# hydradarpa/kalman-hydra

Measured on AMD Instinct MI355X. Metric: frames/sec (Brox flow + EKF update) at 1024^2, higher is better.
Workload: dtype f32 (flow, renders) / f64 (EKF sums and state)

## Files before the change

include/hydra_mi.h:

```cpp
#ifndef HYDRA_MI_H
#define HYDRA_MI_H

#include <stdint.h>

#ifdef __cplusplus
extern "C" {
#endif

#define HM_OK 0
#define HM_ERR_ARG (-1)
#define HM_ERR_HIP (-2)
#define HM_ERR_STATE (-3)
#define HM_ERR_NUMERIC (-4)

const char *hm_last_error(void);
const char *hm_version(void);
int hm_device_count(void);

int hm_dev_alloc(int device, uint64_t bytes, void **out);
int hm_dev_free(int device, void *ptr);
int hm_dev_upload(int device, void *dst, const void *src, uint64_t bytes);
int hm_dev_download(int device, void *dst, const void *src, uint64_t bytes);
int hm_copy_stream_create(int device, void **stream_out);
int hm_copy_stream_destroy(int device, void *stream);
// ... 50 lines not shown
int hm_ctx_destroy(hm_ctx_t h);
int hm_set_texture(hm_ctx_t h, const uint8_t *tex);
int hm_set_observation(hm_ctx_t h, const uint8_t *y_im, const float *y_fx,
                       const float *y_fy, const uint8_t *y_m);
int hm_set_observation_dev(hm_ctx_t h, const uint8_t *d_y_im, const float *d_y_fx,
                           const float *d_y_fy, const uint8_t *d_y_m);

int hm_render(hm_ctx_t h, const double *X, uint8_t *im, float *fx, float *fy, uint8_t *m);


int hm_initjacobian(hm_ctx_t h, const double *X, int masked);
int hm_jz(hm_ctx_t h, const double *Xp, int masked, double *jz, double jzc[4]);
int hm_j(hm_ctx_t h, const double *X, double deltaX, int i, int j, double *out);
int hm_jz_multi(hm_ctx_t h, const double *Xp, int masked, const int32_t *labels, int n_labels,
                double *hz, double *hzc);
int hm_j_multi(hm_ctx_t h, const double *X, double deltaX, int n_pairs, const int32_t *ee,
               const int32_t *labels, int n_labels, double *hsum, double *nz, double *hcomp);
int hm_project_mask(hm_ctx_t h, const uint8_t *y_m, double *X, int *moved);
int hm_prune_mask(hm_ctx_t h, const uint8_t *y_m, uint8_t *out);
int hm_error(hm_ctx_t h, const double *X, int masked, double err[4], float *fx, float *fy);

int hm_measure(hm_ctx_t h, const double *X, double deltaX, int masked,
               double *Hz, double *Hzc, double *HTH);
int hm_update_begin(hm_ctx_t h, const double *W_prior, const double *X0);
int hm_update_prefactor(hm_ctx_t h);
int hm_update_step(hm_ctx_t h, const double *X, double deltaX, int masked, double *step, double *Hzc,
                   double err[4]);
int hm_update_cov(hm_ctx_t h, int which, double *W_out);
int hm_update_run(hm_ctx_t h, const double *W_prior, double *X, double deltaX, int masked, int max_iter,
                  double reltol, int info[4], double *errs, double *Hzc, double *gains, double *W_out);
int hm_cov_fetch(hm_ctx_t h, double *W_out);
int hm_ms_newton(int n_vertices, int n_bars, const int32_t *bars, const double *l0, double kappa, double M,
                 double dt, int maxiter, double tol, double *X, int *newton_iterations);
int hm_ms_worker_create(void **worker);
int hm_ms_worker_destroy(void *worker);
int hm_ms_newton_start(void *worker, int n_vertices, int n_bars, const int32_t *bars, const double *l0, double kappa,
                       double M, double dt, int maxiter, double tol, const double *X);
int hm_ms_newton_finish(void *worker, double *X, int *newton_iterations);
int hm_ms_worker_attach(void *worker, hm_ctx_t ctx);
int hm_newton_dev_start(hm_ctx_t h, int N, int n_bars, const int32_t *bars, const double *l0, double kappa, double M,
                        double dt, int maxiter, double tol, const double *X);
int hm_newton_dev_finish(hm_ctx_t h, double *X, int *newton_iterations);
int hm_update_arm_newton(hm_ctx_t h, void *worker, int n_bars, const int32_t *bars, const double *l0, double kappa,
                         double M, double dt, int maxiter, double tol);
int hm_update_arm_cov(hm_ctx_t h, double eps_F);
int hm_predict_take(hm_ctx_t h, const double *X, int n_bars, const int32_t *bars, const double *l0, double kappa,
// ... 69 lines not shown
```

kalman-hydra_amd/_lib.py:

```python
import ctypes
import os

import numpy as np

_HERE = os.path.dirname(os.path.abspath(__file__))
SO_PATH = os.environ.get("HYDRA_MI_SO") or os.path.join(_HERE, "libhydra_mi.so")

c_f32p = ctypes.POINTER(ctypes.c_float)
c_f64p = ctypes.POINTER(ctypes.c_double)
c_u8p = ctypes.POINTER(ctypes.c_uint8)
c_i32p = ctypes.POINTER(ctypes.c_int32)
c_vp = ctypes.c_void_p

SIGNATURES = {
    "hm_last_error": (ctypes.c_char_p, []),
    "hm_version": (ctypes.c_char_p, []),
    "hm_device_count": (ctypes.c_int, []),
    "hm_dev_alloc": (ctypes.c_int, [ctypes.c_int, ctypes.c_uint64, ctypes.POINTER(c_vp)]),
    "hm_dev_free": (ctypes.c_int, [ctypes.c_int, c_vp]),
    "hm_dev_upload": (ctypes.c_int, [ctypes.c_int, c_vp, c_vp, ctypes.c_uint64]),
    "hm_dev_download": (ctypes.c_int, [ctypes.c_int, c_vp, c_vp, ctypes.c_uint64]),
    "hm_copy_stream_create": (ctypes.c_int, [ctypes.c_int, ctypes.POINTER(c_vp)]),
    "hm_copy_stream_destroy": (ctypes.c_int, [ctypes.c_int, c_vp]),
    "hm_copy_stream_sync": (ctypes.c_int, [ctypes.c_int, c_vp]),
# ... 23 lines not shown
    "hm_op_pyr_down": (ctypes.c_int, [c_vp, ctypes.c_int, ctypes.c_int, ctypes.c_float, c_vp, ctypes.c_int, ctypes.c_int]),
    "hm_op_deriv_all": (ctypes.c_int, [c_vp, c_vp, ctypes.c_int, ctypes.c_int, ctypes.POINTER(c_vp)]),
    "hm_op_add_prolong": (ctypes.c_int, [c_vp, c_vp, c_vp, c_vp, ctypes.c_int, ctypes.c_int, c_vp, c_vp, ctypes.c_int,
                                         ctypes.c_int]),
    "hm_op_warp": (ctypes.c_int, [ctypes.POINTER(c_vp), ctypes.c_int, ctypes.c_int, ctypes.POINTER(c_vp), ctypes.c_int]),
    "hm_op_prepare": (ctypes.c_int, [ctypes.POINTER(c_vp), ctypes.c_int, ctypes.c_int, ctypes.c_float,
                                     ctypes.c_float, ctypes.POINTER(c_vp)]),
    "hm_op_sor": (ctypes.c_int, [c_vp, c_vp, ctypes.POINTER(c_vp), ctypes.c_int, ctypes.c_int, ctypes.c_int,
                                 ctypes.c_int, ctypes.c_float]),
    "hm_ctx_create": (ctypes.c_int, [ctypes.c_int, ctypes.c_int, ctypes.c_int, ctypes.c_int, ctypes.c_int, c_vp,
                                     c_vp, ctypes.c_double, ctypes.c_double, ctypes.c_double, ctypes.POINTER(c_vp)]),
    "hm_ctx_destroy": (ctypes.c_int, [c_vp]),
    "hm_set_texture": (ctypes.c_int, [c_vp, c_vp]),
    "hm_set_observation": (ctypes.c_int, [c_vp, c_vp, c_vp, c_vp, c_vp]),
    "hm_set_observation_dev": (ctypes.c_int, [c_vp, c_vp, c_vp, c_vp, c_vp]),
    "hm_render": (ctypes.c_int, [c_vp, c_vp, c_vp, c_vp, c_vp, c_vp]),
    "hm_initjacobian": (ctypes.c_int, [c_vp, c_vp, ctypes.c_int]),
    "hm_jz": (ctypes.c_int, [c_vp, c_vp, ctypes.c_int, c_f64p, c_f64p]),
    "hm_j": (ctypes.c_int, [c_vp, c_vp, ctypes.c_double, ctypes.c_int, ctypes.c_int, c_f64p]),
    "hm_jz_multi": (ctypes.c_int, [c_vp, c_vp, ctypes.c_int, c_vp, ctypes.c_int, c_vp, c_vp]),
    "hm_j_multi": (ctypes.c_int, [c_vp, c_vp, ctypes.c_double, ctypes.c_int, c_vp, c_vp, ctypes.c_int, c_vp, c_vp, c_vp]),
    "hm_error": (ctypes.c_int, [c_vp, c_vp, ctypes.c_int, c_f64p, c_vp, c_vp]),
    "hm_measure": (ctypes.c_int, [c_vp, c_vp, ctypes.c_double, ctypes.c_int, c_vp, c_vp, c_vp]),
    "hm_update_begin": (ctypes.c_int, [c_vp, c_vp, c_vp]),
    "hm_update_step": (ctypes.c_int, [c_vp, c_vp, ctypes.c_double, ctypes.c_int, c_vp, c_vp, c_f64p]),
    "hm_update_cov": (ctypes.c_int, [c_vp, ctypes.c_int, c_vp]),
    "hm_update_prefactor": (ctypes.c_int, [c_vp]),
    "hm_update_run": (ctypes.c_int, [c_vp, c_vp, c_vp, ctypes.c_double, ctypes.c_int, ctypes.c_int, ctypes.c_double,
                                     ctypes.POINTER(ctypes.c_int), c_vp, c_vp, c_vp, c_vp]),
    "hm_update_last_error": (ctypes.c_int, [c_vp, c_vp, c_f64p]),
    "hm_cov_fetch": (ctypes.c_int, [c_vp, c_vp]),
    "hm_project_mask": (ctypes.c_int, [c_vp, c_vp, c_vp, c_vp]),
    "hm_cov_predict": (ctypes.c_int, [c_vp, c_vp, ctypes.c_int, c_vp, c_vp, ctypes.c_double, ctypes.c_double,
                                      ctypes.c_double, c_vp]),
    "hm_ms_newton": (ctypes.c_int, [ctypes.c_int, ctypes.c_int, c_vp, c_vp, ctypes.c_double, ctypes.c_double,
                                    ctypes.c_double, ctypes.c_int, ctypes.c_double, c_vp, ctypes.POINTER(ctypes.c_int)]),
    "hm_ms_worker_create": (ctypes.c_int, [ctypes.POINTER(c_vp)]),
    "hm_ms_worker_destroy": (ctypes.c_int, [c_vp]),
    "hm_ms_newton_start": (ctypes.c_int, [c_vp, ctypes.c_int, ctypes.c_int, c_vp, c_vp, ctypes.c_double, ctypes.c_double,
                                          ctypes.c_double, ctypes.c_int, ctypes.c_double, c_vp]),
    "hm_ms_newton_finish": (ctypes.c_int, [c_vp, c_vp, ctypes.POINTER(ctypes.c_int)]),
    "hm_ms_worker_attach": (ctypes.c_int, [c_vp, c_vp]),
    "hm_newton_dev_start": (ctypes.c_int, [c_vp, ctypes.c_int, ctypes.c_int, c_vp, c_vp, ctypes.c_double, ctypes.c_double,
                                           ctypes.c_double, ctypes.c_int, ctypes.c_double, c_vp]),
    "hm_newton_dev_finish": (ctypes.c_int, [c_vp, c_vp, ctypes.POINTER(ctypes.c_int)]),
    "hm_prune_mask": (ctypes.c_int, [c_vp, c_vp, c_vp]),
# ... 154 lines not shown
```

kalman-hydra_amd/csrc/ekf.hip:

```cpp
#include "hm_common.h"
#include "ekf_kernels.h"
#include "dense_kernels.h"
#include "chol_flow_kernels.h"
#include "project_kernels.h"
#include "predict_kernels.h"
#include "view_kernels.h"
#include "body_kernels.h"
#include "roi_kernels.h"
#include "smooth_kernels.h"
#include <algorithm>
#include <atomic>
#include <chrono>
#include <cmath>
#include <condition_variable>
#include <cstring>
#include <functional>
#include <mutex>
#include <set>
#include <thread>
#include <utility>
#include <vector>

struct Helper {
    std::thread th;
// ... 50 lines not shown

struct hm_ctx {
    int device, W, H, N, T, E, njobs;
    HmOwner own{1};
    Helper helper;
    bool helper_used = false;
    int tail_async = 1;
    double eps_Z, eps_J, eps_M;
    hipStream_t stream;
    int *d_tri, *d_star_off, *d_star_tri, *d_edges;
    int *d_nb_off = nullptr, *d_nb_u = nullptr, *d_nb_e = nullptr;
    float *d_uv;
    uint8_t *d_tex;
    std::vector<int> edges;
    uint8_t *d_yim, *d_ym;
    float *d_yfx, *d_yfy, *d_yfxm, *d_yfym;
    bool obs_owned = true;
    const uint8_t *o_yim, *o_ym;
    const float *o_yfx, *o_yfy;
    bool have_tex, have_obs, have_ref;
    Targets ref, P, Q;
    TriSetup *d_setup, *d_cfgs;
    int4 *d_ubox;
    int *d_tlist = nullptr, *d_tcount = nullptr;
    unsigned *d_tmask = nullptr;
    double *d_X, *d_out, *d_partial;
    uint8_t *d_im8, *d_m8;
    std::vector<double> X0;
    double *d_HTH;
    double *d_H, *d_Hz, *d_Hzc, *d_invW0, *d_Af[2], *d_T[2], *d_step, *d_Wtmp, *d_X0, *d_Xn, *d_Wprior, *d_gain, *d_Awork, *d_Lt[2];
    std::vector<double> upd_X0;
    int upd_last = -1, upd_prev = -1;
    double *d_Wres;
    double *pin;
    size_t pin_n;
    int *pin_scratch;
    std::vector<double> resv, tailv;
    int result_delay = 0;
    bool tail_pending = false;
    bool tail_valid = false;
    long long tail_ticket = 0;
    hipStream_t tail_stream = nullptr;
    const uint8_t *armed_mask = nullptr;
    std::vector<int> sp_h_off, sp_h_bar, sp_h_other;
    std::vector<double> sp_h_blk;
    std::vector<int32_t> sp_bars_cached;
// ... 326 lines not shown
                hm_set_error("hm_ctx_create: vertex %d has %d neighbours, limit %d", v, (int)nb[v].size(), PREP_MAX_ENTRIES / 4 - 1);
                rc = HM_ERR_ARG;
            }
        }
        step(upload(h->own, &h->d_nb_off, noff.data(), noff.size()));
        step(upload(h->own, &h->d_nb_u, nu.data(), nu.size()));
        step(upload(h->own, &h->d_nb_e, ne.data(), ne.size()));
    }
    hipError_t e = hipSuccess;
    auto dev = [&](auto **p, size_t bytes) { if (e == hipSuccess) e = h->own.alloc(p, bytes); };
    if (rc == HM_OK) {
        const char *pe = getenv("HYDRA_MI_EKF_PRIORITY");
        e = h->own.stream(&h->stream, !(pe && atoi(pe) == 0));
        dev(&h->d_tex, n);
        dev(&h->d_yim, n);
        dev(&h->d_ym, n);
        dev(&h->d_yfx, n * sizeof(float));
        dev(&h->d_yfy, n * sizeof(float));
        dev(&h->d_yfxm, n * sizeof(float));
        dev(&h->d_yfym, n * sizeof(float));
        dev(&h->d_setup, (size_t)T * sizeof(TriSetup));
        dev(&h->d_cfgs, (size_t)N * MEAS_NCFG * (EKF_MAX_STAR + 1) * sizeof(TriSetup));
        dev(&h->d_ubox, (size_t)N * UBOX_STRIDE * sizeof(int4));
        dev(&h->d_tmask, (size_t)N * TMASK_STRIDE * sizeof(unsigned));
        dev(&h->d_tlist, (size_t)N * TMASK_STRIDE * sizeof(int));
        dev(&h->d_tcount, (size_t)N * sizeof(int));
        dev(&h->d_X, (size_t)4 * N * sizeof(double));
        dev(&h->d_out, (size_t)h->njobs * MEAS_VSPLIT_MAX * MEAS_OUT * sizeof(double));
        dev(&h->d_partial, (size_t)h->red_blocks * 4 * sizeof(double));
        h->ntiles = hm_cdiv(W, RI_W) * hm_cdiv(H, 8);
        dev(&h->d_tpart, (size_t)h->ntiles * RI_NV * sizeof(double));
        dev(&h->d_im8, n);
        dev(&h->d_m8, n);
        const size_t n4 = (size_t)4 * N, nn = n4 * n4 * sizeof(double);
        dev(&h->d_H, nn);
        dev(&h->d_HTH, nn);
        if (e == hipSuccess) e = hipMemsetAsync(h->d_HTH, 0, nn, h->stream);
        dev(&h->d_invW0, nn);
        const size_t nn_aug = (size_t)(hm_cdiv((int)n4, DNB) * DNB + DNB) * n4 * sizeof(double);
        dev(&h->d_Af[0], nn_aug);
        dev(&h->d_Af[1], nn_aug);
        dev(&h->d_Awork, nn_aug);
        const size_t ld_bytes = (size_t)hm_cdiv((int)n4, DNB) * DNB * DNB * sizeof(double);
        dev(&h->d_T[0], nn);
        dev(&h->d_T[1], nn);
        dev(&h->d_step, n4 * sizeof(double));
// ... 62 lines not shown
        HM_ARG(value >= 2 && value <= 2048, "hm_ctx_tune: chol_flow_wgs must be in 2..2048 (the chain workgroup and at least one task workgroup)");
        h->flow_wgs = value;
    } else if (!strcmp(key, "render_rows")) {
        HM_ARG(value == 8 || value == 16, "hm_ctx_tune: render_rows must be 8 or 16");
        h->render_rows = value;
    } else if (!strcmp(key, "chol_flow_stall")) {
        HM_ARG(value >= 0 && value <= 100000, "hm_ctx_tune: chol_flow_stall must be in 0..100000");
        h->flow_stall = value;
    } else if (!strcmp(key, "result_delay")) {
        HM_ARG(value >= 0 && value <= 5000, "hm_ctx_tune: result_delay must be in 0..5000 (microseconds)");
        h->result_delay = value;
    } else if (!strcmp(key, "tail_async")) {
        HM_ARG(value == 0 || value == 1, "hm_ctx_tune: tail_async must be 0 or 1");
        h->tail_async = value;
    } else if (!strcmp(key, "tail_split")) {
        HM_ARG(value == 0 || value == 1, "hm_ctx_tune: tail_split must be 0 or 1");
        h->tail_split = value;
    } else if (!strcmp(key, "newton_fail")) {
        HM_ARG(value == 0 || value == 1, "hm_ctx_tune: newton_fail must be 0 or 1");
        h->newton_fail = value;
    } else if (!strcmp(key, "speculate")) {
        HM_ARG(value == 0 || value == 1, "hm_ctx_tune: speculate must be 0 or 1");
        h->speculate = value;
    } else if (!strcmp(key, "edge_split")) {
        HM_ARG(value >= 1 && value <= MEAS_VSPLIT_MAX, "hm_ctx_tune: edge_split must be in 1..%d", MEAS_VSPLIT_MAX);
        h->esplit = value;
    } else if (!strcmp(key, "body_stats_cap")) {
        HM_ARG(value >= 1 && value <= BODY_STATS_CAP, "hm_ctx_tune: body_stats_cap must be in 1..%d", BODY_STATS_CAP);
        h->stats_cap = value;
    } else if (!strcmp(key, "body_rec_chunk")) {
        HM_ARG(value >= 0, "hm_ctx_tune: body_rec_chunk must be >= 0 (0: the default size)");
        h->rec_chunk = value;
    } else {
        hm_set_error("hm_ctx_tune: unknown key '%s'", key);
        return HM_ERR_ARG;
    }
    return HM_OK;
}
extern "C" void *hm_ctx_stream(hm_ctx_t h)
{
    (void)ctx_join(h);
    return h ? (void *)h->stream : nullptr;
}
extern "C" int hm_ctx_sync(hm_ctx_t h)
{
    HM_ARG(h != nullptr, "hm_ctx_sync: NULL handle");
// ... 405 lines not shown
    const int n = h->W * h->H;
    if (fx) HM_HIP(hipMemcpyAsync(fx, h->P.fx, (size_t)n * sizeof(float), hipMemcpyDeviceToHost, h->stream));
    if (fy) HM_HIP(hipMemcpyAsync(fy, h->P.fy, (size_t)n * sizeof(float), hipMemcpyDeviceToHost, h->stream));
    HM_HIP(hipMemcpyAsync(h->h_tpart.data(), h->d_tpart, (size_t)render_strips(h) * RI_NV * sizeof(double), hipMemcpyDeviceToHost, h->stream));
    HM_HIP(stream_wait(h->stream));
    double s6[RI_NV];
    hm_tile_partial_sums(h->h_tpart.data(), render_strips(h), s6);
    for (int k = 0; k < 4; k++) err[k] = s6[k];
    return HM_OK;
}

static int measure_dev(hm_ctx *h, const double *dX, bool ref_ready, double deltaX, int masked, bool regions_ready = false,
                       bool scatter = true)
{
    if (!ref_ready) {
        int rc = render_iter(h, dX, h->ref, false, masked, !regions_ready, deltaX);
        if (rc) return rc;
        regions_ready = true;
    }
    MeasureArgs a;
    measure_args(h, dX, deltaX, masked, a);
    if (!regions_ready) hipLaunchKernelGGL(k_star_regions, dim3(h->N), dim3(REGION_NT), 0, h->stream, a, h->d_area);
    hipLaunchKernelGGL(k_measure_vertex, dim3(h->N, h->vsplit), dim3(MEAS_NT), 0, h->stream, a,
                       (const TriSetup *)h->d_cfgs, (const int4 *)h->d_ubox, (const unsigned *)h->d_tmask);
    if (h->E > 0) hipLaunchKernelGGL(k_measure_edge, dim3(h->E, h->esplit), dim3(MEAS_NT), 0, h->stream, a);
    if (scatter) {
        ScatterArgs s = {h->d_out, h->d_edges, h->N, h->E, h->vsplit, h->esplit, h->eps_Z, h->eps_J, h->eps_M, deltaX, h->d_HTH, h->d_Hz, h->d_Hzc};
        hipLaunchKernelGGL(k_hth_scatter, dim3(hm_cdiv(h->njobs, 4)), dim3(256), 0, h->stream, s);
    }
    HM_HIP(hipGetLastError());
    return HM_OK;
}

static void measure_args(hm_ctx *h, const double *dX, double deltaX, int masked, MeasureArgs &a)
{
    a.m = Mesh{h->W, h->H, h->N, h->T, h->d_tri, h->d_uv, h->d_tex};
    a.topo = StarTopo{h->d_star_off, h->d_star_tri, h->d_edges, h->E};
    a.ref = h->ref;
    a.obs = obs_of(h, masked);
    a.X = dX;
    a.delta = deltaX;
    a.out = h->d_out;
    a.pool = h->pool;
    a.vsplit = h->vsplit;
    a.esplit = h->esplit;
    a.iZ = 1.0 / h->eps_Z; a.iJ = 1.0 / h->eps_J; a.iM = 1.0 / h->eps_M;
    a.cfgs = h->d_cfgs;
    a.ubox = h->d_ubox;
    a.tmask = h->d_tmask;
    a.tlist = h->d_tlist;
    a.tcount = h->d_tcount;
    a.tmask_stride = TMASK_STRIDE;
}

static int measure_on_device(hm_ctx *h, const double *X, double deltaX, int masked, bool scatter = true)
{
    HM_HIP(hipMemcpyAsync(h->d_X, X, (size_t)4 * h->N * sizeof(double), hipMemcpyHostToDevice, h->stream));
    h->X0.assign(X, X + 4 * h->N);
    h->have_ref = true;
    return measure_dev(h, h->d_X, false, deltaX, masked, false, scatter);
}

extern "C" int hm_measure(hm_ctx_t h, const double *X, double deltaX, int masked, double *Hz, double *Hzc, double *HTH)
{
    HM_ARG(h && X && Hz && HTH, "hm_measure: NULL argument");
    HM_JOIN(h);
    HM_ARG(deltaX > 0, "hm_measure: deltaX must be positive");
    NEED_TEX(h, "hm_measure");
    NEED_OBS(h, "hm_measure");
    HM_HIP(hipSetDevice(h->device));
    const size_t n4 = (size_t)4 * h->N;
    int *ovf = h->pin_scratch;
    for (int attempt = 0;; attempt++) {
        int rc = measure_on_device(h, X, deltaX, masked);
        if (rc) return rc;
        *ovf = 0;
        HM_HIP(hipMemcpyAsync(ovf, h->pool.overflow, sizeof(int), hipMemcpyDeviceToHost, h->stream));
        HM_HIP(hipStreamSynchronize(h->stream));
        if (!*ovf) break;
        if (attempt) { hm_set_error("hm_measure: the star regions do not fit the difference-image pool"); return HM_ERR_STATE; }
        rc = pool_grow(h, "hm_measure");
        if (rc) return rc;
    }
    HM_HIP(hipMemcpyAsync(Hz, h->d_Hz, n4 * sizeof(double), hipMemcpyDeviceToHost, h->stream));
    if (Hzc) HM_HIP(hipMemcpyAsync(Hzc, h->d_Hzc, n4 * 4 * sizeof(double), hipMemcpyDeviceToHost, h->stream));
    HM_HIP(hipMemcpyAsync(HTH, h->d_HTH, n4 * n4 * sizeof(double), hipMemcpyDeviceToHost, h->stream));
    HM_HIP(hipStreamSynchronize(h->stream));
    return HM_OK;
}

static int aug_rows(int n) { return hm_cdiv(n, DNB) * DNB + DNB; }

static void chol_factor(hm_ctx *h, double *A, double *L, double *Lt, double *T, double *M, int n, bool with_rhs,
                        bool first_done = false, hipStream_t st = nullptr)
{
    if (!st) st = h->stream;
    const int nb = hm_cdiv(n, DNB);
    const int nrows = with_rhs ? aug_rows(n) : n;
    const int nbr = hm_cdiv(nrows, DNB);
    if (h->chol_flow) {
        FlowArgs a = {A, L, Lt, T, h->d_flowP, n, nrows, nb, nbr, h->d_flowctl, h->flow_stall};
        if (!first_done) hipLaunchKernelGGL(k_flow_fill, dim3(nrows + FLOW_FILL_WGS), dim3(256), 0, st, a);
        hipLaunchKernelGGL(k_chol_flow, dim3(h->flow_wgs), dim3(FLOW_NT), 0, st, a);
        return;
    }
    if (!first_done) hipLaunchKernelGGL(k_chol_first, dim3(1), dim3(64), 0, st, A, Lt, n);
    for (int k = 0; k < nb; k++) {
        const int mr = nbr - k - 1, mc = std::max(nb - k - 1, 1);
        hipLaunchKernelGGL(k_chol_step, dim3((mc + k + 1) * (mr + 1)), dim3(256), 0, st, A, L, Lt, T, M, n, nrows, nb, k, mc, mc + k + 1, mr + 1);
    }
// ... 2077 lines not shown
```

kalman-hydra_amd/csrc/ekf_kernels.h:

```cpp
#pragma once
#include <hip/hip_runtime.h>
#include <stdint.h>

#define EKF_SUB 256
#define EKF_MAX_STAR 24
#define EKF_TILE 16
#define EKF_MAX_TRI 4096

struct TriSetup {
    double ea[3], eb[3], ec[3];
    double ecb[3];
    int cmin, cmax, rmin, rmax;
    int tl[3];
    float inv;
    int i0, i1, i2;
    float ux[3], uy[3], ax[3], ay[3];
};

__device__ __forceinline__ void d_tri_attr(TriSetup &s, const float *__restrict__ uv, const double *__restrict__ X, int N)
{
    const int id[3] = {s.i0, s.i1, s.i2};
    for (int k = 0; k < 3; k++) {
        s.ux[k] = uv[2 * id[k]];
        s.uy[k] = uv[2 * id[k] + 1];
// ... 468 lines not shown
{
    P.xi[pp] = make_short2(POOL_EMPTY, 0); P.yi[pp] = make_short2(0, 0);
    P.xfx[pp] = 0.0f; P.xfy[pp] = 0.0f; P.yfx[pp] = 0.0f; P.yfy[pp] = 0.0f;
    P.vxfx[pp] = 0.0f; P.vyfy[pp] = 0.0f;
}

struct MeasureArgs {
    Mesh m;
    StarTopo topo;
    Targets ref;
    Obs obs;
    const double *X;
    double delta;
    double *out;
    DPool pool;
    int vsplit;
    int esplit;
    double iZ, iJ, iM;
    TriSetup *cfgs;
    int4 *ubox;
    unsigned *tmask;
    int *tlist, *tcount;
    int tmask_stride;
};

#define MEAS_NT 256
#define MEAS_OUT 40
#define MEAS_VSPLIT_MAX 16
enum {
    A_X = 0, A_Y = 4, A_VX = 8, A_VY = 9,
    A_XX = 10, A_XY = 11, A_YY = 12,
    A_XVX = 13, A_YVX = 14,
    A_XVY = 15, A_YVY = 16,
    A_VXVX = 17, A_VYVY = 18,
    A_NV = 19
};
enum {
    B_XX = 0, B_XY = 1, B_YX = 2, B_YY = 3,
    B_XVX = 4, B_YVX = 5, B_VXX = 6, B_VXY = 7, B_VXVX = 8,
    B_XVY = 9, B_YVY = 10, B_VYX = 11, B_VYY = 12, B_VYVY = 13,
    B_NV = 14
};

#define MEAS_NCFG 5
#define UBOX_STRIDE (EKF_MAX_STAR + 4)
#define TMASK_STRIDE 1024

__device__ inline void d_vertex_cfgs(TriSetup (*cfg)[EKF_MAX_STAR + 1], int nsv, const int *trv, const Mesh &m,
                                     const double *X, int v, double d, int nthreads)
{
    const int wv = threadIdx.x >> 6, lane = threadIdx.x & 63, nw = nthreads >> 6;
    const double dxs[MEAS_NCFG] = {0, d, -d, 0, 0}, dys[MEAS_NCFG] = {0, 0, 0, d, -d};
    for (int c = wv; c < MEAS_NCFG; c += nw) d_star_setups(cfg[c], nsv, trv, m, X, v, dxs[c], dys[c], lane, 64);
}

#define REGION_NT (64 * MEAS_NCFG)
struct RegionShared {
    int4 tbox[MEAS_NCFG][EKF_MAX_STAR + 1];
    double ea[MEAS_NCFG][EKF_MAX_STAR + 1][3], eb[MEAS_NCFG][EKF_MAX_STAR + 1][3], ecb[MEAS_NCFG][EKF_MAX_STAR + 1][3];
    int box[MEAS_NCFG][4];
    int reg[4];
    int wsum[8];
};
template <int NT>
__device__ inline void d_star_regions(const MeasureArgs &a, int *__restrict__ area, int v, RegionShared &sh)
{
    const Mesh &m = a.m;
    const int nsv = a.topo.star_off[v + 1] - a.topo.star_off[v];
    const int *trv = a.topo.star_tri + a.topo.star_off[v];
    const int wv = threadIdx.x >> 6, lane = threadIdx.x & 63;
    constexpr int NW = NT / 64;
    const double d = a.delta;
    const double dxs[MEAS_NCFG] = {0, d, -d, 0, 0}, dys[MEAS_NCFG] = {0, 0, 0, d, -d};
    for (int cf = wv; cf < MEAS_NCFG; cf += NW) {
        TriSetup *dst = a.cfgs + ((size_t)v * MEAS_NCFG + cf) * (EKF_MAX_STAR + 1);
        if (lane < nsv) {
            TriSetup su;
            d_star_setup_one(su, trv[lane], m, a.X, v, dxs[cf], dys[cf]);
            dst[lane] = su;
            sh.tbox[cf][lane] = make_int4(su.cmin, su.cmax, su.rmin, su.rmax);
            for (int k = 0; k < 3; k++) { sh.ea[cf][lane][k] = su.ea[k]; sh.eb[cf][lane][k] = su.eb[k]; sh.ecb[cf][lane][k] = su.ecb[k]; }
        }
        if ((nsv & 1) && lane == 0) {
            TriSetup pad;
            d_star_setup_pad(pad);
            pad.inv = 0.0f; pad.i0 = pad.i1 = pad.i2 = 0;
            for (int k = 0; k < 3; k++) { pad.ux[k] = pad.uy[k] = pad.ax[k] = pad.ay[k] = 0.0f; }
            dst[nsv] = pad;
        }
    }
    __syncthreads();
    if (wv == 0 && lane < UBOX_STRIDE) {
        int4 u = make_int4(1, 0, 1, 0);
        if (lane < nsv)
            for (int cfg = 0; cfg < MEAS_NCFG; cfg++) {
                const int4 s = sh.tbox[cfg][lane];
                if (s.x > s.y) continue;
                if (u.x > u.y) u = s;
                else u = make_int4(min(u.x, s.x), max(u.y, s.y), min(u.z, s.z), max(u.w, s.w));
            }
        a.ubox[(size_t)v * UBOX_STRIDE + lane] = u;
    }
    for (int cf = wv; cf < MEAS_NCFG; cf += NW) {
        int c0 = m.W, c1 = -1, r0 = m.H, r1 = -1;
        if (lane < nsv) {
            const int4 s = sh.tbox[cf][lane];
            if (s.x <= s.y) { c0 = s.x; c1 = s.y; r0 = s.z; r1 = s.w; }
        }
        for (int o = 16; o > 0; o >>= 1) {
            c0 = min(c0, __shfl_down(c0, o, 64)); c1 = max(c1, __shfl_down(c1, o, 64));
            r0 = min(r0, __shfl_down(r0, o, 64)); r1 = max(r1, __shfl_down(r1, o, 64));
        }
        if (lane == 0) { sh.box[cf][0] = c0; sh.box[cf][1] = c1; sh.box[cf][2] = r0; sh.box[cf][3] = r1; }
    }
// ... 67 lines not shown
                                     long long &tot, long long *s )
{
    long long a = 0, b = 0, c = 0;
    for (int i = threadIdx.x; i < N; i += NT) {
        const long long x = area[i];
        c += x;
        if (i < v) a += x;
        if (i < w) b += x;
    }
    for (int o = 32; o > 0; o >>= 1) {
        a += __shfl_down(a, o, 64); b += __shfl_down(b, o, 64); c += __shfl_down(c, o, 64);
    }
    const int lane = threadIdx.x & 63, wv = threadIdx.x >> 6;
    if (lane == 0) { s[wv * 3] = a; s[wv * 3 + 1] = b; s[wv * 3 + 2] = c; }
    __syncthreads();
    bv = 0; bw = 0; tot = 0;
    for (int k = 0; k < NT / 64; k++) { bv += s[k * 3]; bw += s[k * 3 + 1]; tot += s[k * 3 + 2]; }
}

#ifndef MEAS_OCC
#define MEAS_OCC 4
#endif
__global__ __launch_bounds__(MEAS_NT, MEAS_OCC) void k_measure_vertex(MeasureArgs a, const TriSetup *__restrict__ cfgs,
                                                                const int4 *__restrict__ ubox, const unsigned *__restrict__ tmask)
{
    __shared__ double s_red[(MEAS_NT / 64) * MEAS_OUT];
    __shared__ double s_k255[511];
    const double *k255 = s_k255 + 255;
    d_fill_k255(s_k255, MEAS_NT);
    const Mesh &m = a.m;
    const int N = m.N, W = m.W;
    const int v = blockIdx.x, job = v;
    const double *X = a.X;
    const double d = a.delta;
    const int nsv = a.topo.star_off[v + 1] - a.topo.star_off[v];
    const TriSetup *__restrict__ s_cfg[MEAS_NCFG];
#pragma unroll
    for (int c = 0; c < MEAS_NCFG; c++) s_cfg[c] = cfgs + ((size_t)v * MEAS_NCFG + c) * (EKF_MAX_STAR + 1);
    __syncthreads();
    const int c0 = a.pool.hdr[4 * v], r0 = a.pool.hdr[4 * v + 1], rw = a.pool.hdr[4 * v + 2], rh = a.pool.hdr[4 * v + 3];
    __shared__ long long s_sum[(MEAS_NT / 64) * 3];
    long long base, unused, total;
    d_region_sums<MEAS_NT>(a.pool.area, N, v, 0, base, unused, total, s_sum);
    const bool park = total <= a.pool.cap;
    if (v == 0 && blockIdx.y == 0 && threadIdx.x == 0) *a.pool.overflow = park ? 0 : 1;
    double acc[A_NV];
#pragma unroll
    for (int k = 0; k < A_NV; k++) acc[k] = 0.0;
    const int wave = __builtin_amdgcn_readfirstlane(threadIdx.x >> 6);
    const int lx = threadIdx.x & 7, ly = (threadIdx.x & 63) >> 3;
    const int ntx = (rw + 7) >> 3, ntiles = ntx * ((rh + 7) >> 3);
    const int nwaves = (MEAS_NT / 64) * gridDim.y;
    const int listed = a.tcount[v];
    const int nwalk = listed >= 0 ? listed : ntiles;
    for (int j = blockIdx.y * (MEAS_NT / 64) + wave; j < nwalk; j += nwaves) {
        const int tile = listed >= 0 ? a.tlist[(size_t)v * a.tmask_stride + j] : j;
        const int tr0 = r0 + 8 * (tile / ntx), tc0 = c0 + 8 * (tile % ntx);
        const int r = tr0 + ly, c = tc0 + lx;
        unsigned mask = 0;
        if (listed >= 0) {
            mask = tmask[(size_t)v * a.tmask_stride + tile];
        } else {
            for (int k = 0; k < nsv; k++) {
                const int4 b = ubox[(size_t)v * UBOX_STRIDE + k];
                if (!((b.y < tc0) | (b.x > tc0 + 7) | (b.w < tr0) | (b.z > tr0 + 7))) mask |= 1u << k;
            }
        }
        const long long pp = base + (long long)tile * 64 + (threadIdx.x & 63);
        if (c >= W || r >= m.H) {
            if (park) d_park_empty(a.pool, pp);
            continue;
        }
        const int p = r * W + c;
        const int racc = a.ref.acc[p], rcnt = a.ref.cnt[p];
        const float rfx = a.ref.fx[p], rfy = a.ref.fy[p];
        StarVel vel, none;
        StarTex q0, q1, q2, q3, q4;
        StarVal sref = d_star_eval<true>(s_cfg[0], mask, c, r, m, v, (float)(X[2 * N + 2 * v] + d),
                                         (float)(X[2 * N + 2 * v] - d), (float)(-(X[2 * N + 2 * v + 1] + d)),
                                         (float)(-(X[2 * N + 2 * v + 1] - d)), vel, q0);
        StarVal sxp = d_star_eval<false>(s_cfg[1], mask, c, r, m, v, 0, 0, 0, 0, none, q1);
        StarVal sxm = d_star_eval<false>(s_cfg[2], mask, c, r, m, v, 0, 0, 0, 0, none, q2);
        StarVal syp = d_star_eval<false>(s_cfg[3], mask, c, r, m, v, 0, 0, 0, 0, none, q3);
        StarVal sym = d_star_eval<false>(s_cfg[4], mask, c, r, m, v, 0, 0, 0, 0, none, q4);
        {
            const int e0 = d_star_texels(m.tex, q0), e1 = d_star_texels(m.tex, q1), e2 = d_star_texels(m.tex, q2);
            const int e3 = d_star_texels(m.tex, q3), e4 = d_star_texels(m.tex, q4);
            sref.acc += e0; sxp.acc += e1; sxm.acc += e2; syp.acc += e3; sym.acc += e4;
        }
        const bool covered = sref.cnt + sxp.cnt + sxm.cnt + syp.cnt + sym.cnt != 0;
        const bool tile_live = __any(covered);
        if (park && (threadIdx.x & 63) == __builtin_ctzll(__builtin_amdgcn_read_exec()))
            a.pool.live[base / 64 + tile] = tile_live ? 1 : 0;
        if (!covered) {
            if (park) d_park_empty(a.pool, pp);
            continue;
        }
        const StarVal svxp = {sref.acc, sref.cnt, vel.fxp, sref.fy}, svxm = {sref.acc, sref.cnt, vel.fxm, sref.fy};
        const StarVal svyp = {sref.acc, sref.cnt, sref.fx, vel.fyp}, svym = {sref.acc, sref.cnt, sref.fx, vel.fym};
        const Diff dxp = d_diff(k255, racc, rcnt, rfx, rfy, sref, sxp), dxm = d_diff(k255, racc, rcnt, rfx, rfy, sref, sxm);
        const Diff dyp = d_diff(k255, racc, rcnt, rfx, rfy, sref, syp), dym = d_diff(k255, racc, rcnt, rfx, rfy, sref, sym);
        const Diff dvxp = d_diff(k255, racc, rcnt, rfx, rfy, sref, svxp), dvxm = d_diff(k255, racc, rcnt, rfx, rfy, sref, svxm);
        const Diff dvyp = d_diff(k255, racc, rcnt, rfx, rfy, sref, svyp), dvym = d_diff(k255, racc, rcnt, rfx, rfy, sref, svym);
        const int rim = racc > 255 ? 255 : racc, rm = rcnt > 0 ? 255 : 0;
        const double z = k255[(int)a.obs.yim[p] - rim];
        const double zm = d_q255(k255, 255 * (int)a.obs.ym[p] - rm);
        const double zfx = (double)(a.obs.yfx[p] - rfx), zfy = (double)(a.obs.yfy[p] + rfy);
// ... 418 lines not shown
```

Baseline: 334.1.

## Share edge functions across the five perturbed star configurations in vertex measurement

```diff
diff --git a/include/hydra_mi.h b/include/hydra_mi.h
--- a/include/hydra_mi.h
+++ b/include/hydra_mi.h
@@ -96,6 +96,9 @@
 
 int hm_measure(hm_ctx_t h, const double *X, double deltaX, int masked,
                double *Hz, double *Hzc, double *HTH);
+int hm_measure_fill(hm_ctx_t h, int byte);
+int hm_measure_raw(hm_ctx_t h, int32_t dims[4], double *out, int32_t *hdr, int32_t *area, int32_t *live,
+                   uint32_t *planes, long long cap);
 int hm_update_begin(hm_ctx_t h, const double *W_prior, const double *X0);
 int hm_update_prefactor(hm_ctx_t h);
 int hm_update_step(hm_ctx_t h, const double *X, double deltaX, int masked, double *step, double *Hzc,
diff --git a/kalman-hydra_amd/_lib.py b/kalman-hydra_amd/_lib.py
--- a/kalman-hydra_amd/_lib.py
+++ b/kalman-hydra_amd/_lib.py
@@ -69,6 +69,8 @@
     "hm_j_multi": (ctypes.c_int, [c_vp, c_vp, ctypes.c_double, ctypes.c_int, c_vp, c_vp, ctypes.c_int, c_vp, c_vp, c_vp]),
     "hm_error": (ctypes.c_int, [c_vp, c_vp, ctypes.c_int, c_f64p, c_vp, c_vp]),
     "hm_measure": (ctypes.c_int, [c_vp, c_vp, ctypes.c_double, ctypes.c_int, c_vp, c_vp, c_vp]),
+    "hm_measure_fill": (ctypes.c_int, [c_vp, ctypes.c_int]),
+    "hm_measure_raw": (ctypes.c_int, [c_vp, c_vp, c_vp, c_vp, c_vp, c_vp, c_vp, ctypes.c_longlong]),
     "hm_update_begin": (ctypes.c_int, [c_vp, c_vp, c_vp]),
     "hm_update_step": (ctypes.c_int, [c_vp, c_vp, ctypes.c_double, ctypes.c_int, c_vp, c_vp, c_f64p]),
     "hm_update_cov": (ctypes.c_int, [c_vp, ctypes.c_int, c_vp]),
diff --git a/kalman-hydra_amd/csrc/ekf.hip b/kalman-hydra_amd/csrc/ekf.hip
--- a/kalman-hydra_amd/csrc/ekf.hip
+++ b/kalman-hydra_amd/csrc/ekf.hip
@@ -96,6 +96,9 @@
     Targets ref, P, Q;
     TriSetup *d_setup, *d_cfgs;
     int4 *d_ubox;
+    StarShare *d_share = nullptr;
+    int *d_share_ok = nullptr;
+    int shared_edges = 1;
     int *d_tlist = nullptr, *d_tcount = nullptr;
     unsigned *d_tmask = nullptr;
     double *d_X, *d_out, *d_partial;
@@ -468,6 +471,8 @@
         dev(&h->d_setup, (size_t)T * sizeof(TriSetup));
         dev(&h->d_cfgs, (size_t)N * MEAS_NCFG * (EKF_MAX_STAR + 1) * sizeof(TriSetup));
         dev(&h->d_ubox, (size_t)N * UBOX_STRIDE * sizeof(int4));
+        dev(&h->d_share, (size_t)N * EKF_MAX_STAR * sizeof(StarShare));
+        dev(&h->d_share_ok, (size_t)N * sizeof(int));
         dev(&h->d_tmask, (size_t)N * TMASK_STRIDE * sizeof(unsigned));
         dev(&h->d_tlist, (size_t)N * TMASK_STRIDE * sizeof(int));
         dev(&h->d_tcount, (size_t)N * sizeof(int));
@@ -576,6 +581,9 @@
     } else if (!strcmp(key, "speculate")) {
         HM_ARG(value == 0 || value == 1, "hm_ctx_tune: speculate must be 0 or 1");
         h->speculate = value;
+    } else if (!strcmp(key, "shared_edges")) {
+        HM_ARG(value == 0 || value == 1, "hm_ctx_tune: shared_edges must be 0 or 1");
+        h->shared_edges = value;
     } else if (!strcmp(key, "edge_split")) {
         HM_ARG(value >= 1 && value <= MEAS_VSPLIT_MAX, "hm_ctx_tune: edge_split must be in 1..%d", MEAS_VSPLIT_MAX);
         h->esplit = value;
@@ -1027,7 +1035,8 @@
     measure_args(h, dX, deltaX, masked, a);
     if (!regions_ready) hipLaunchKernelGGL(k_star_regions, dim3(h->N), dim3(REGION_NT), 0, h->stream, a, h->d_area);
     hipLaunchKernelGGL(k_measure_vertex, dim3(h->N, h->vsplit), dim3(MEAS_NT), 0, h->stream, a,
-                       (const TriSetup *)h->d_cfgs, (const int4 *)h->d_ubox, (const unsigned *)h->d_tmask);
+                       (const TriSetup *)h->d_cfgs, (const int4 *)h->d_ubox, (const unsigned *)h->d_tmask,
+                       (const StarShare *)h->d_share);
     if (h->E > 0) hipLaunchKernelGGL(k_measure_edge, dim3(h->E, h->esplit), dim3(MEAS_NT), 0, h->stream, a);
     if (scatter) {
         ScatterArgs s = {h->d_out, h->d_edges, h->N, h->E, h->vsplit, h->esplit, h->eps_Z, h->eps_J, h->eps_M, deltaX, h->d_HTH, h->d_Hz, h->d_Hzc};
@@ -1056,6 +1065,9 @@
     a.tlist = h->d_tlist;
     a.tcount = h->d_tcount;
     a.tmask_stride = TMASK_STRIDE;
+    a.share = h->d_share;
+    a.share_ok = h->d_share_ok;
+    a.shared_edges = h->shared_edges;
 }
 
 static int measure_on_device(hm_ctx *h, const double *X, double deltaX, int masked, bool scatter = true)
@@ -1091,6 +1103,55 @@
     if (Hzc) HM_HIP(hipMemcpyAsync(Hzc, h->d_Hzc, n4 * 4 * sizeof(double), hipMemcpyDeviceToHost, h->stream));
     HM_HIP(hipMemcpyAsync(HTH, h->d_HTH, n4 * n4 * sizeof(double), hipMemcpyDeviceToHost, h->stream));
     HM_HIP(hipStreamSynchronize(h->stream));
+    return HM_OK;
+}
+
+extern "C" int hm_measure_fill(hm_ctx_t h, int byte)
+{
+    HM_ARG(h != nullptr, "hm_measure_fill: NULL argument");
+    HM_JOIN(h);
+    HM_HIP(hipSetDevice(h->device));
+    const size_t pc = (size_t)h->pool.cap;
+    HM_HIP(hipMemsetAsync(h->d_out, byte, (size_t)h->njobs * MEAS_VSPLIT_MAX * MEAS_OUT * sizeof(double), h->stream));
+    if (pc) {
+        HM_HIP(hipMemsetAsync(h->pool.live, byte, (pc / 64 + 1) * sizeof(int), h->stream));
+        for (short2 *q : {h->pool.xi, h->pool.yi}) HM_HIP(hipMemsetAsync(q, byte, pc * sizeof(short2), h->stream));
+        for (float *q : {h->pool.xfx, h->pool.xfy, h->pool.yfx, h->pool.yfy, h->pool.vxfx, h->pool.vyfy})
+            HM_HIP(hipMemsetAsync(q, byte, pc * sizeof(float), h->stream));
+    }
+    HM_HIP(hipStreamSynchronize(h->stream));
+    return HM_OK;
+}
+extern "C" int hm_measure_raw(hm_ctx_t h, int32_t dims[4], double *out, int32_t *hdr, int32_t *area, int32_t *live,
+                              uint32_t *planes, long long cap)
+{
+    HM_ARG(h != nullptr, "hm_measure_raw: NULL argument");
+    HM_JOIN(h);
+    HM_HIP(hipSetDevice(h->device));
+    HM_HIP(hipStreamSynchronize(h->stream));
+    if (dims) {
+        std::vector<int> ok(h->N);
+        HM_HIP(hipMemcpy(ok.data(), h->d_share_ok, (size_t)h->N * sizeof(int), hipMemcpyDeviceToHost));
+        dims[0] = h->njobs; dims[1] = h->vsplit; dims[2] = h->esplit; dims[3] = 0;
+        for (int x : ok) dims[3] += x != 0;
+    }
+    std::vector<int> ar(h->N);
+    HM_HIP(hipMemcpy(ar.data(), h->d_area, (size_t)h->N * sizeof(int), hipMemcpyDeviceToHost));
+    long long total = 0;
+    for (int x : ar) total += x;
+    if (area) memcpy(area, ar.data(), (size_t)h->N * sizeof(int));
+    if (out) HM_HIP(hipMemcpy(out, h->d_out, (size_t)h->njobs * MEAS_VSPLIT_MAX * MEAS_OUT * sizeof(double), hipMemcpyDeviceToHost));
+    if (hdr) HM_HIP(hipMemcpy(hdr, h->pool.hdr, (size_t)4 * h->N * sizeof(int), hipMemcpyDeviceToHost));
+    if (live || planes) {
+        HM_ARG(total <= cap, "hm_measure_raw: the star regions hold %lld pixels, the caller has room for %lld", total, cap);
+        if (total > h->pool.cap) { hm_set_error("hm_measure_raw: the last measurement did not fit the pool"); return HM_ERR_STATE; }
+    }
+    const size_t tp = (size_t)total;
+    if (live && tp) HM_HIP(hipMemcpy(live, h->pool.live, tp / 64 * sizeof(int), hipMemcpyDeviceToHost));
+    if (planes && tp) {
+        const void *src[8] = {h->pool.xi, h->pool.yi, h->pool.xfx, h->pool.xfy, h->pool.yfx, h->pool.yfy, h->pool.vxfx, h->pool.vyfy};
+        for (int k = 0; k < 8; k++) HM_HIP(hipMemcpy(planes + (size_t)k * (size_t)cap, src[k], tp * 4, hipMemcpyDeviceToHost));
+    }
     return HM_OK;
 }
 
diff --git a/kalman-hydra_amd/csrc/ekf_kernels.h b/kalman-hydra_amd/csrc/ekf_kernels.h
--- a/kalman-hydra_amd/csrc/ekf_kernels.h
+++ b/kalman-hydra_amd/csrc/ekf_kernels.h
@@ -514,6 +514,9 @@
     unsigned *tmask;
     int *tlist, *tcount;
     int tmask_stride;
+    struct StarShare *share;
+    int *share_ok;
+    int shared_edges;
 };
 
 #define MEAS_NT 256
@@ -536,6 +539,15 @@
 
 #define MEAS_NCFG 5
 #define UBOX_STRIDE (EKF_MAX_STAR + 4)
+
+struct StarShare {
+    double ea[3], eb[3], ec[3];
+    double bx[2], by[2];
+    double cf[MEAS_NCFG - 1][2];
+    double thr0, thr[MEAS_NCFG][2];
+    float inv[MEAS_NCFG];
+    int opp;
+};
 #define TMASK_STRIDE 1024
 
 __device__ inline void d_vertex_cfgs(TriSetup (*cfg)[EKF_MAX_STAR + 1], int nsv, const int *trv, const Mesh &m,
@@ -550,10 +562,112 @@
 struct RegionShared {
     int4 tbox[MEAS_NCFG][EKF_MAX_STAR + 1];
     double ea[MEAS_NCFG][EKF_MAX_STAR + 1][3], eb[MEAS_NCFG][EKF_MAX_STAR + 1][3], ecb[MEAS_NCFG][EKF_MAX_STAR + 1][3];
+    float inv[MEAS_NCFG][EKF_MAX_STAR + 1];
+    int meta[MEAS_NCFG][EKF_MAX_STAR + 1];
     int box[MEAS_NCFG][4];
     int reg[4];
     int wsum[8];
 };
+__device__ inline void d_star_share(const MeasureArgs &a, const RegionShared &sh, int v, int nsv, const int *trv, int lane)
+{
+    const Mesh &m = a.m;
+    bool ok = true;
+    if (lane < nsv) {
+        const int t = trv[lane];
+        const int m0 = sh.meta[0][lane];
+        const bool turned = (m0 & 8) != 0;
+        const int i0 = m.tri[3 * t], i1 = m.tri[3 * t + (turned ? 2 : 1)], i2 = m.tri[3 * t + (turned ? 1 : 2)];
+        const long long x0 = d_snap(a.X[2 * i0]), y0 = d_snap(a.X[2 * i0 + 1]), x1 = d_snap(a.X[2 * i1]), y1 = d_snap(a.X[2 * i1 + 1]);
+        const long long x2 = d_snap(a.X[2 * i2]), y2 = d_snap(a.X[2 * i2 + 1]);
+        const int opp = i0 == v ? 0 : (i1 == v ? 1 : 2), j1 = (opp + 1) % 3, j2 = (opp + 2) % 3;
+        auto pick = [](int k, long long q0, long long q1, long long q2) { return k == 0 ? q0 : (k == 1 ? q1 : q2); };
+        const long long vx = pick(opp, x0, x1, x2), vy = pick(opp, y0, y1, y2);
+        const double d = a.delta;
+        const long long vxp = d_snap(a.X[2 * v] + d), vxm = d_snap(a.X[2 * v] + (-d));
+        const long long vyp = d_snap(a.X[2 * v + 1] + d), vym = d_snap(a.X[2 * v + 1] + (-d));
+        const long long lim = (long long)1 << 24;
+        for (long long q : {x0, y0, x1, y1, x2, y2, vxp, vxm, vyp, vym}) ok &= q > -lim && q < lim;
+        StarShare s;
+        const int order[3] = {opp, j1, j2};
+        for (int i = 0; i < 3; i++) {
+            const int k = order[i];
+            s.ea[i] = sh.ea[0][lane][k]; s.eb[i] = sh.eb[0][lane][k];
+            s.ec[i] = sh.ecb[0][lane][k] - (double)((m0 >> k) & 1);
+        }
+        s.bx[0] = (double)(128 - pick(j2, x0, x1, x2)); s.by[0] = (double)(128 - pick(j2, y0, y1, y2));
+        s.bx[1] = (double)(128 - pick(j1, x0, x1, x2)); s.by[1] = (double)(128 - pick(j1, y0, y1, y2));
+        const double dxp = (double)(vxp - vx), dxm = (double)(vxm - vx), dyp = (double)(vyp - vy), dym = (double)(vym - vy);
+        s.cf[0][0] = dxp; s.cf[0][1] = -dxp; s.cf[1][0] = dxm; s.cf[1][1] = -dxm;
+        s.cf[2][0] = -dyp; s.cf[2][1] = dyp; s.cf[3][0] = -dym; s.cf[3][1] = dym;
+        s.thr0 = -(double)((m0 >> opp) & 1);
+        for (int cf = 0; cf < MEAS_NCFG; cf++) {
+            const int mc = sh.meta[cf][lane];
+            s.thr[cf][0] = -(double)((mc >> j1) & 1); s.thr[cf][1] = -(double)((mc >> j2) & 1);
+            s.inv[cf] = sh.inv[cf][lane];
+            ok &= sh.inv[cf][lane] != 0.0f && ((mc ^ m0) & 8) == 0 && (((mc ^ m0) >> opp) & 1) == 0;
+        }
+        s.opp = opp;
+        a.share[(size_t)v * EKF_MAX_STAR + lane] = s;
+    }
+    const bool all_ok = __all(ok) && m.W <= 65536 && m.H <= 65536;
+    if (lane == 0) a.share_ok[v] = all_ok ? 1 : 0;
+}
+
+struct StarVal5 {
+    StarVal s[MEAS_NCFG];
+    StarTex q[MEAS_NCFG];
+};
+__device__ __forceinline__ void d_star_eval5(const StarShare *__restrict__ share, const TriSetup *__restrict__ geo, unsigned mask,
+                                             int c, int r, const Mesh &m, int v, float vxp, float vxm, float nvyp, float nvym,
+                                             StarVel &vel, StarVal5 &o)
+{
+#pragma unroll
+    for (int k = 0; k < MEAS_NCFG; k++) { o.s[k] = StarVal{0, 0, 0.0f, 0.0f}; o.q[k].t0 = -1; o.q[k].t1 = -1; }
+    vel.fxp = 0.0f; vel.fxm = 0.0f; vel.fyp = 0.0f; vel.fym = 0.0f;
+    const double dc = (double)c, dr = (double)r;
+    for (unsigned mm = mask; mm != 0; mm &= mm - 1) {
+        const int k = __builtin_ctz(mm);
+        const StarShare &h = share[k];
+        const TriSetup &t = geo[k];
+        auto add = [&](StarVal &s, StarTex &q, double p0, double p1, double p2, float inv, bool with_vel) {
+            const float f0 = (float)p0, f1 = (float)p1, f2 = (float)p2;
+            const float l1 = (h.opp == 0 ? f1 : (h.opp == 1 ? f0 : f2)) * inv;
+            const float l2 = (h.opp == 0 ? f2 : (h.opp == 1 ? f1 : f0)) * inv;
+            const int at = d_texel_at(t, l1, l2, m.W, m.H);
+            if (s.cnt == 0) q.t0 = at;
+            else if (s.cnt == 1) q.t1 = at;
+            else s.acc += m.tex[at];
+            const float a0 = t.ax[0], a1 = t.ax[1], a2 = t.ax[2];
+            const float b0 = t.ay[0], b1 = t.ay[1], b2 = t.ay[2];
+            s.fx = s.fx + d_lerp(a0, a1, a2, l1, l2);
+            s.fy = s.fy + d_lerp(b0, b1, b2, l1, l2);
+            s.cnt++;
+            if (with_vel) {
+                const bool v0 = t.i0 == v, v1 = t.i1 == v, v2 = t.i2 == v;
+                vel.fxp = vel.fxp + d_lerp(v0 ? vxp : a0, v1 ? vxp : a1, v2 ? vxp : a2, l1, l2);
+                vel.fxm = vel.fxm + d_lerp(v0 ? vxm : a0, v1 ? vxm : a1, v2 ? vxm : a2, l1, l2);
+                vel.fyp = vel.fyp + d_lerp(v0 ? nvyp : b0, v1 ? nvyp : b1, v2 ? nvyp : b2, l1, l2);
+                vel.fym = vel.fym + d_lerp(v0 ? nvym : b0, v1 ? nvym : b1, v2 ? nvym : b2, l1, l2);
+            }
+        };
+        const double e0 = fma(h.ea[0], dc, fma(h.eb[0], dr, h.ec[0]));
+        const double r1 = fma(h.ea[1], dc, fma(h.eb[1], dr, h.ec[1]));
+        const double r2 = fma(h.ea[2], dc, fma(h.eb[2], dr, h.ec[2]));
+        const bool in0 = e0 > h.thr0;
+        if (in0 & (r1 > h.thr[0][0]) & (r2 > h.thr[0][1])) add(o.s[0], o.q[0], e0, r1, r2, h.inv[0], true);
+#pragma unroll
+        for (int ax = 0; ax < 2; ax++) {
+            const double q1 = fma((double)EKF_SUB, ax ? dc : dr, ax ? h.bx[0] : h.by[0]);
+            const double q2 = fma((double)EKF_SUB, ax ? dc : dr, ax ? h.bx[1] : h.by[1]);
+#pragma unroll
+            for (int cf = 1 + 2 * ax; cf < 3 + 2 * ax; cf++) {
+                const double e1 = fma(h.cf[cf - 1][0], q1, r1), e2 = fma(h.cf[cf - 1][1], q2, r2);
+                if (in0 & (e1 > h.thr[cf][0]) & (e2 > h.thr[cf][1])) add(o.s[cf], o.q[cf], e0, e1, e2, h.inv[cf], false);
+            }
+        }
+    }
+}
+
 template <int NT>
 __device__ inline void d_star_regions(const MeasureArgs &a, int *__restrict__ area, int v, RegionShared &sh)
 {
@@ -572,6 +686,8 @@
             dst[lane] = su;
             sh.tbox[cf][lane] = make_int4(su.cmin, su.cmax, su.rmin, su.rmax);
             for (int k = 0; k < 3; k++) { sh.ea[cf][lane][k] = su.ea[k]; sh.eb[cf][lane][k] = su.eb[k]; sh.ecb[cf][lane][k] = su.ecb[k]; }
+            sh.inv[cf][lane] = su.inv;
+            sh.meta[cf][lane] = su.tl[0] | (su.tl[1] << 1) | (su.tl[2] << 2) | (su.i1 != m.tri[3 * trv[lane] + 1] ? 8 : 0);
         }
         if ((nsv & 1) && lane == 0) {
             TriSetup pad;
@@ -582,6 +698,7 @@
         }
     }
     __syncthreads();
+    if (wv == 1) d_star_share(a, sh, v, nsv, trv, lane);
     if (wv == 0 && lane < UBOX_STRIDE) {
         int4 u = make_int4(1, 0, 1, 0);
         if (lane < nsv)
@@ -695,7 +812,8 @@
 #define MEAS_OCC 4
 #endif
 __global__ __launch_bounds__(MEAS_NT, MEAS_OCC) void k_measure_vertex(MeasureArgs a, const TriSetup *__restrict__ cfgs,
-                                                                const int4 *__restrict__ ubox, const unsigned *__restrict__ tmask)
+                                                                const int4 *__restrict__ ubox, const unsigned *__restrict__ tmask,
+                                                                const StarShare *__restrict__ share)
 {
     __shared__ double s_red[(MEAS_NT / 64) * MEAS_OUT];
     __shared__ double s_k255[511];
@@ -710,6 +828,8 @@
     const TriSetup *__restrict__ s_cfg[MEAS_NCFG];
 #pragma unroll
     for (int c = 0; c < MEAS_NCFG; c++) s_cfg[c] = cfgs + ((size_t)v * MEAS_NCFG + c) * (EKF_MAX_STAR + 1);
+    const StarShare *__restrict__ s_share = share + (size_t)v * EKF_MAX_STAR;
+    const bool shared = a.shared_edges != 0 && a.share_ok[v] != 0;
     __syncthreads();
     const int c0 = a.pool.hdr[4 * v], r0 = a.pool.hdr[4 * v + 1], rw = a.pool.hdr[4 * v + 2], rh = a.pool.hdr[4 * v + 3];
     __shared__ long long s_sum[(MEAS_NT / 64) * 3];
@@ -739,23 +859,31 @@
                 if (!((b.y < tc0) | (b.x > tc0 + 7) | (b.w < tr0) | (b.z > tr0 + 7))) mask |= 1u << k;
             }
         }
+        if (c >= W || r >= m.H) {
+            if (park) d_park_empty(a.pool, base + (long long)tile * 64 + (threadIdx.x & 63));
+            continue;
+        }
+        StarVel vel, none;
+        StarTex q0, q1, q2, q3, q4;
+        StarVal sref, sxp, sxm, syp, sym;
+        const float vxp = (float)(X[2 * N + 2 * v] + d), vxm = (float)(X[2 * N + 2 * v] - d);
+        const float nvyp = (float)(-(X[2 * N + 2 * v + 1] + d)), nvym = (float)(-(X[2 * N + 2 * v + 1] - d));
+        if (shared) {
+            StarVal5 o;
+            d_star_eval5(s_share, s_cfg[0], mask, c, r, m, v, vxp, vxm, nvyp, nvym, vel, o);
+            sref = o.s[0]; sxp = o.s[1]; sxm = o.s[2]; syp = o.s[3]; sym = o.s[4];
+            q0 = o.q[0]; q1 = o.q[1]; q2 = o.q[2]; q3 = o.q[3]; q4 = o.q[4];
+        } else {
+            sref = d_star_eval<true>(s_cfg[0], mask, c, r, m, v, vxp, vxm, nvyp, nvym, vel, q0);
+            sxp = d_star_eval<false>(s_cfg[1], mask, c, r, m, v, 0, 0, 0, 0, none, q1);
+            sxm = d_star_eval<false>(s_cfg[2], mask, c, r, m, v, 0, 0, 0, 0, none, q2);
+            syp = d_star_eval<false>(s_cfg[3], mask, c, r, m, v, 0, 0, 0, 0, none, q3);
+            sym = d_star_eval<false>(s_cfg[4], mask, c, r, m, v, 0, 0, 0, 0, none, q4);
+        }
         const long long pp = base + (long long)tile * 64 + (threadIdx.x & 63);
-        if (c >= W || r >= m.H) {
-            if (park) d_park_empty(a.pool, pp);
-            continue;
-        }
         const int p = r * W + c;
         const int racc = a.ref.acc[p], rcnt = a.ref.cnt[p];
         const float rfx = a.ref.fx[p], rfy = a.ref.fy[p];
-        StarVel vel, none;
-        StarTex q0, q1, q2, q3, q4;
-        StarVal sref = d_star_eval<true>(s_cfg[0], mask, c, r, m, v, (float)(X[2 * N + 2 * v] + d),
-                                         (float)(X[2 * N + 2 * v] - d), (float)(-(X[2 * N + 2 * v + 1] + d)),
-                                         (float)(-(X[2 * N + 2 * v + 1] - d)), vel, q0);
-        StarVal sxp = d_star_eval<false>(s_cfg[1], mask, c, r, m, v, 0, 0, 0, 0, none, q1);
-        StarVal sxm = d_star_eval<false>(s_cfg[2], mask, c, r, m, v, 0, 0, 0, 0, none, q2);
-        StarVal syp = d_star_eval<false>(s_cfg[3], mask, c, r, m, v, 0, 0, 0, 0, none, q3);
-        StarVal sym = d_star_eval<false>(s_cfg[4], mask, c, r, m, v, 0, 0, 0, 0, none, q4);
         {
             const int e0 = d_star_texels(m.tex, q0), e1 = d_star_texels(m.tex, q1), e2 = d_star_texels(m.tex, q2);
             const int e3 = d_star_texels(m.tex, q3), e4 = d_star_texels(m.tex, q4);
```

Result: no change. 335.3 (median of 6 runs) (+0.4%).
